# eniac/flamingo

Hardware: AMD Instinct MI355X
Metric: device-resident aggregate+unmask GB/s, N clients × L int32 per round (higher is better)
Workload: dtype u32

## Files before the change

flamingo_amd/csrc/flm_internal.h:

```cpp
#pragma once
#include <stdint.h>
#include <stddef.h>
#include <hip/hip_runtime.h>

#include "flm_host_layout.h"
#include "flm_items.h"

namespace flm {

constexpr uint32_t kAbcd = 0x64636261u;
constexpr uint32_t kSigma0 = 0x61707865u, kSigma1 = 0x3320646eu, kSigma2 = 0x79622d32u,
                   kSigma3 = 0x6b206574u;

hipError_t launch_seed_schedule(const uint8_t *d_seeds, const int8_t *d_signs, int K, SeedRec *d_recs,
                                uint32_t *d_meta, hipStream_t stream, uint32_t *d_zero = nullptr,
                                uint64_t zero_n = 0);
int seed_schedule_groups(int K, uint64_t zero_n);
hipError_t launch_items(int subtiles, int variant, const Item *d_items, int n_items, const uint32_t *d_rows,
                        uint64_t row_pitch, const SeedRec *d_recs, const uint32_t *d_meta,
                        uint32_t *d_out, hipStream_t stream);
int small_round_slots(int B);
hipError_t launch_small_round(int B, const uint32_t *d_rows, uint64_t pitch, int N, const uint8_t *d_seeds,
                              const int8_t *d_signs, int K, uint64_t L, uint64_t mask_lo, uint64_t mask_hi,
                              uint32_t ctr0, uint32_t *d_out, uint32_t *d_meta, hipStream_t stream);
hipError_t launch_small_client_mask(const uint32_t *d_x, uint64_t pitch, int N, const int64_t *d_seg,
                                   const uint8_t *d_seeds, const int8_t *d_signs, uint64_t L, uint32_t bias,
                                   uint32_t *d_out, hipStream_t stream);
uint32_t pair_units_count(int K, uint64_t L, uint32_t *n_tiles);
hipError_t launch_pair_units(bool side, const SeedRec *d_recs, int K, uint32_t *d_dst, uint64_t L, uint32_t *d_ws,
                             int groups, hipStream_t stream);
hipError_t launch_flag_set(uint32_t *d_ws, hipStream_t stream);
hipError_t launch_prg_expand(const SeedRec *d_recs, int K, uint64_t L, uint64_t pitch, uint32_t ctr0,
                             uint32_t *d_out, int groups, hipStream_t stream);
hipError_t launch_add2(const uint32_t *d_a, const uint32_t *d_b, uint32_t *d_dst, uint64_t n, hipStream_t stream);
constexpr int kMaxParts = 16;
struct PartPtrs {
    const uint32_t *p[kMaxParts];
};
hipError_t launch_shard_sum(const uint32_t *const *d_parts, int G, uint64_t lo, uint64_t n, uint32_t *d_dst,
                            hipStream_t stream);
hipError_t launch_chacha20_xor(const uint32_t key[8], const uint32_t nonce[2], uint64_t counter,
                               const uint8_t *d_in, uint8_t *d_out, size_t n, hipStream_t stream);

// ... 70 lines not shown
```

flamingo_amd/csrc/flm_kernels.hip:

```cpp
#include "flm_internal.h"

namespace flm {

#define FLM_ROTL(v, c) __builtin_rotateleft32((v), (c))
#define FLM_QR(a, b, c, d)                       \
    a += b; d ^= a; d = FLM_ROTL(d, 16);          \
    c += d; b ^= c; b = FLM_ROTL(b, 12);          \
    a += b; d ^= a; d = FLM_ROTL(d, 8);           \
    c += d; b ^= c; b = FLM_ROTL(b, 7);

#define FLM_GAP_A1 ""
#define FLM_GAP_AX ""
#define FLM_GAP_X1 ""
#define FLM_GAP_XR ""
#define FLM_GAP_R0 "s_nop 1\n\t"
#define FLM_GAP_R1 "s_nop 1\n\t"
#define FLM_GAP_R2 "s_nop 1\n\t"
#define FLM_GAP_RA "s_nop 2\n\t"
#define FLM_S_A(a, b) "v_add_u32 %[" #a "], %[" #b "], %[" #a "]\n\t"
#define FLM_S_X(a, b) "v_xor_b32 %[" #a "], %[" #b "], %[" #a "]\n\t"
#define FLM_S_R(a, s) "v_alignbit_b32 %[" #a "], %[" #a "], %[" #a "], " #s "\n\t"
#define FLM_S_STEP(a, b, c, d, s)                                                                       \
    FLM_S_A(a##0, b##0) FLM_S_A(a##1, b##1) FLM_GAP_A1 FLM_S_A(a##2, b##2) FLM_S_A(a##3, b##3) FLM_GAP_AX \
    FLM_S_X(d##0, a##0) FLM_S_X(d##1, a##1) FLM_GAP_X1 FLM_S_X(d##2, a##2) FLM_S_X(d##3, a##3) FLM_GAP_XR \
// ... 54 lines not shown
#pragma unroll
        for (int i = 0; i < 10; ++i) r.pad[i] = 0;
        recs[k] = r;
    }
    __shared__ uint32_t s_cnt[2][4];
    const unsigned long long bn = __ballot(neg != 0), bb = __ballot(bad != 0);
    const int w = threadIdx.x >> 6;
    if ((threadIdx.x & 63) == 0) { s_cnt[0][w] = __popcll(bn); s_cnt[1][w] = __popcll(bb); }
    __syncthreads();
    if (threadIdx.x == 0) {
        meta[2 + 2 * blockIdx.x] = s_cnt[0][0] + s_cnt[0][1] + s_cnt[0][2] + s_cnt[0][3];
        meta[3 + 2 * blockIdx.x] = s_cnt[1][0] + s_cnt[1][1] + s_cnt[1][2] + s_cnt[1][3];
        if (blockIdx.x == 0) meta[0] = gridDim.x;
    }
}

__device__ __forceinline__ uint32_t meta_nneg(const uint32_t *__restrict__ meta) {
    const uint32_t parts = meta[0];
    uint32_t n = 0;
    for (uint32_t p = 0; p < parts; ++p) n += meta[2 + 2 * p];
    return n;
}

__device__ __forceinline__ void chacha_mask_add(const SeedRec *__restrict__ rec, uint32_t ctr,
                                                uint32_t (&m)[16]) {
    const uint32_t k0 = rec->k[0], k1 = rec->k[1], k2 = rec->k[2], k3 = rec->k[3];
    const uint32_t k4 = rec->k[4], k5 = rec->k[5], k6 = rec->k[6], k7 = rec->k[7];
    const uint32_t xc = rec->xorc;
    uint32_t x0, x1, x2, x3, x4, x5, x6, x7, x8, x9, x10, x11, x12, x13, x14, x15;
    x0 = rec->a0;
    x12 = FLM_ROTL(ctr ^ x0, 16);
    x8 = k4 + x12;
    x4 = FLM_ROTL(k0 ^ x8, 12);
    x0 += x4;
    x12 = FLM_ROTL(x12 ^ x0, 8);
    x8 += x12;
    x4 = FLM_ROTL(x4 ^ x8, 7);
    x1 = rec->col1[0]; x5 = rec->col1[1]; x9 = rec->col1[2]; x13 = rec->col1[3];
    x2 = rec->col2[0]; x6 = rec->col2[1]; x10 = rec->col2[2]; x14 = rec->col2[3];
    x3 = rec->col3[0]; x7 = rec->col3[1]; x11 = rec->col3[2]; x15 = rec->col3[3];
    FLM_QR4(x0, x5, x10, x15, x1, x6, x11, x12, x2, x7, x8, x13, x3, x4, x9, x14);
#pragma unroll
    for (int r = 0; r < 9; ++r) {
        FLM_QR4(x0, x4, x8, x12, x1, x5, x9, x13, x2, x6, x10, x14, x3, x7, x11, x15);
        FLM_QR4(x0, x5, x10, x15, x1, x6, x11, x12, x2, x7, x8, x13, x3, x4, x9, x14);
    }
    m[0] += (x0 + kSigma0) ^ xc;
    m[1] += (x1 + kSigma1) ^ xc;
    m[2] += (x2 + kSigma2) ^ xc;
    m[3] += (x3 + kSigma3) ^ xc;
    m[4] += (x4 + k0) ^ xc;
    m[5] += (x5 + k1) ^ xc;
    m[6] += (x6 + k2) ^ xc;
    m[7] += (x7 + k3) ^ xc;
    m[8] += (x8 + k4) ^ xc;
    m[9] += (x9 + k5) ^ xc;
    m[10] += (x10 + k6) ^ xc;
    m[11] += (x11 + k7) ^ xc;
    m[12] += (x12 + ctr) ^ xc;
    m[13] += x13 ^ xc;
    m[14] += x14 ^ xc;
    m[15] += x15 ^ xc;
}

typedef uint32_t u32x4 __attribute__((ext_vector_type(4)));

template <bool BL, int AUX = 0>
__device__ __forceinline__ void load_row(const uint32_t *base, uint32_t bytes, int lane, u32x4 (&v)[4]) {
    const __amdgpu_buffer_rsrc_t rs = __builtin_amdgcn_make_buffer_rsrc(const_cast<uint32_t *>(base), 0,
                                                                        (int)bytes, 0x00020000);
#pragma unroll
    for (int j = 0; j < 4; ++j)
        v[j] = __builtin_bit_cast(
            u32x4, __builtin_amdgcn_raw_buffer_load_b128(rs, BL ? 64 * lane + 16 * j : 16 * lane + 1024 * j, 0, AUX));
}

template <int S>
__device__ __forceinline__ void reduce_out(const u32x4 *__restrict__ lds, uint32_t *__restrict__ out,
                                           uint64_t base, int valid, uint32_t bias, bool atomic) {
    constexpr int Cw = kWavesPerGroup / S;
    if (!atomic) {
        for (int q = threadIdx.x; q < S * 256; q += kThreads) {
            const int s = q >> 8, p = q & 255;
            u32x4 acc = u32x4(bias);
#pragma unroll
            for (int c = 0; c < Cw; ++c) acc = acc + lds[(s + S * c) * 256 + p];
            const int slot = s * kWaveSlots + 4 * p;
            uint32_t *dst = out + base + slot;
            if (slot + 3 < valid) {
                *reinterpret_cast<u32x4 *>(dst) = acc;
            } else {
                if (slot + 0 < valid) dst[0] = acc.x;
                if (slot + 1 < valid) dst[1] = acc.y;
                if (slot + 2 < valid) dst[2] = acc.z;
            }
        }
    } else {
        const uint32_t *l32 = reinterpret_cast<const uint32_t *>(lds);
        for (int d = threadIdx.x; d < S * kWaveSlots; d += kThreads) {
            const int s = d >> 10, o = d & 1023;
            uint32_t acc = bias;
#pragma unroll
            for (int c = 0; c < Cw; ++c) acc += l32[(s + S * c) * 1024 + o];
            const int slot = s * kWaveSlots + o;
            if (slot < valid) atomicAdd(out + base + slot, acc);
        }
    }
}

template <int S, bool BL, bool MERGED, int WPE, int RUM = 2, int AUX = 0, bool SPREAD = false>
__global__ __launch_bounds__(kThreads, WPE) void items_kernel(const Item *__restrict__ items,
                                                              const uint32_t *__restrict__ rows,
                                                              uint64_t row_pitch,
                                                              const SeedRec *__restrict__ recs,
                                                              const uint32_t *__restrict__ meta,
                                                              uint32_t *__restrict__ out) {
    static_assert(!MERGED || BL, "merged accumulation needs block-layout rows");
    constexpr int Cw = kWavesPerGroup / S;
    constexpr int RU = MERGED ? RUM : 4;
    __shared__ u32x4 lds[kWavesPerGroup * 256];
    __shared__ uint32_t claim[S];

    const Item it = items[blockIdx.x];
    const int lane = threadIdx.x & 63;
    const int w = __builtin_amdgcn_readfirstlane(threadIdx.x >> 6);
    const int s = w % S, c = w / S;
    if constexpr (!SPREAD && Cw > 1) {
        if (threadIdx.x < S) claim[threadIdx.x] = 0u;
        __syncthreads();
    }
    const uint32_t flags = it.flags;
    const bool has_rows = flags & kHasRows, has_mask = flags & kHasMask;

    u32x4 racc[4] = {u32x4(0u), u32x4(0u), u32x4(0u), u32x4(0u)};
    uint32_t m[16];
#pragma unroll
    for (int i = 0; i < 16; ++i) m[i] = 0;

    uint32_t nr = 0, ns = 0, r0 = 0, q0 = 0;
    if (has_rows) {
        r0 = (uint32_t)(((uint64_t)it.nrows * c) / Cw);
        nr = (uint32_t)(((uint64_t)it.nrows * (c + 1)) / Cw) - r0;
    }
    if (has_mask) {
        q0 = it.k0 + (uint32_t)(((uint64_t)it.nseeds * c) / Cw);
        ns = it.k0 + (uint32_t)(((uint64_t)it.nseeds * (c + 1)) / Cw) - q0;
    }
    const int sub_slot = s * kWaveSlots;
    const int row_valid = (int)it.row_valid - sub_slot;
    const uint32_t row_bytes =
        row_valid >= kWaveSlots ? 4u * kWaveSlots : (row_valid > 0 ? 16u * (uint32_t)((row_valid + 3) / 4) : 0u);
    const uint32_t *rp = rows + it.row_in + (uint64_t)r0 * row_pitch + sub_slot;
    const uint32_t ctr = (uint32_t)(it.mask_ctr + (uint64_t)(sub_slot / 16) + (uint64_t)lane);
    const SeedRec *rec = recs + q0;
    if (row_valid <= 0) nr = 0;

    auto add_row = [&](const u32x4 (&v)[4]) {
        if constexpr (MERGED) {
#pragma unroll
            for (int j = 0; j < 4; ++j) {
                m[4 * j + 0] += v[j].x; m[4 * j + 1] += v[j].y; m[4 * j + 2] += v[j].z; m[4 * j + 3] += v[j].w;
            }
        } else {
#pragma unroll
            for (int j = 0; j < 4; ++j) racc[j] = racc[j] + v[j];
        }
    };

    if constexpr (SPREAD) {
        uint32_t q = 0;
        for (uint32_t r = 0; r < nr; ++r) {
            u32x4 v[4];
            load_row<BL, AUX>(rp, row_bytes, lane, v);
            if (q < ns && (uint64_t)q * nr <= (uint64_t)r * ns) {
                chacha_mask_add(rec, ctr, m);
                ++rec;
                ++q;
            }
            add_row(v);
            rp += row_pitch;
        }
        for (; q < ns; ++q) {
            chacha_mask_add(rec, ctr, m);
            ++rec;
        }
    } else if constexpr (Cw > 1) {
        const uint32_t NR = (has_rows && row_valid > 0) ? it.nrows : 0u;
        const uint32_t NS = has_mask ? it.nseeds : 0u;
        const uint32_t *rb = rows + it.row_in + sub_slot;
        const uint32_t caddr = (uint32_t)(uintptr_t)(__attribute__((address_space(3))) uint32_t *)&claim[s];
        auto next = [&]() -> uint32_t {
            uint32_t v = 0;
            if (lane == 0)
                asm volatile("ds_add_rtn_u32 %0, %1, %2\n\ts_waitcnt lgkmcnt(0)" : "=v"(v) : "v"(caddr), "v"(1u) : "memory");
            return __builtin_amdgcn_readlane(v, 0);
        };
        const uint32_t NP = NR < NS ? NR : NS;
        uint32_t i = next();
        for (; i < NP; i = next()) {
            u32x4 v4[4];
            load_row<BL, AUX>(rb + (uint64_t)i * row_pitch, row_bytes, lane, v4);
            chacha_mask_add(recs + it.k0 + i, ctr, m);
            add_row(v4);
        }
        for (; i < NS; i = next()) chacha_mask_add(recs + it.k0 + i, ctr, m);
        if (NR > NS) {
            const uint32_t a = NS + (uint32_t)(((uint64_t)(NR - NS) * c) / Cw);
            const uint32_t b = NS + (uint32_t)(((uint64_t)(NR - NS) * (c + 1)) / Cw);
            const uint32_t *rq = rb + (uint64_t)a * row_pitch;
            uint32_t rr = b - a;
            for (; rr >= RU; rr -= RU) {
                u32x4 v4[RU][4];
#pragma unroll
                for (int u = 0; u < RU; ++u) load_row<BL, AUX>(rq + u * row_pitch, row_bytes, lane, v4[u]);
#pragma unroll
                for (int u = 0; u < RU; ++u) add_row(v4[u]);
                rq += RU * row_pitch;
            }
            for (; rr > 0; --rr) {
                u32x4 v4[4];
                load_row<BL, AUX>(rq, row_bytes, lane, v4);
                add_row(v4);
                rq += row_pitch;
            }
        }
    } else {
        const uint32_t np = nr < ns ? nr : ns;
        for (uint32_t q = 0; q < np; ++q) {
            u32x4 v[4];
            load_row<BL, AUX>(rp, row_bytes, lane, v);
            chacha_mask_add(rec, ctr, m);
            add_row(v);
            rp += row_pitch;
            ++rec;
        }
        uint32_t rr = nr - np;
        for (; rr >= RU; rr -= RU) {
            u32x4 v[RU][4];
#pragma unroll
            for (int u = 0; u < RU; ++u) load_row<BL, AUX>(rp + u * row_pitch, row_bytes, lane, v[u]);
#pragma unroll
            for (int u = 0; u < RU; ++u) add_row(v[u]);
            rp += RU * row_pitch;
        }
        for (; rr > 0; --rr) {
            u32x4 v[4];
            load_row<BL, AUX>(rp, row_bytes, lane, v);
            add_row(v);
            rp += row_pitch;
        }
        for (uint32_t q = np; q < ns; ++q) {
            chacha_mask_add(rec, ctr, m);
            ++rec;
        }
    }

    u32x4 *R = lds + w * 256;
    const uint32_t mbias = it.mask_bias + ((flags & kMaskBiasNneg) ? meta_nneg(meta) : 0u);
    if constexpr (MERGED) {
        R[4 * lane + 0] = u32x4{m[0], m[1], m[2], m[3]};
        R[4 * lane + 1] = u32x4{m[4], m[5], m[6], m[7]};
        R[4 * lane + 2] = u32x4{m[8], m[9], m[10], m[11]};
        R[4 * lane + 3] = u32x4{m[12], m[13], m[14], m[15]};
        __syncthreads();
        const uint64_t base = has_mask ? it.mask_out : it.row_out;
        const int valid = has_mask ? (int)it.mask_valid : (int)it.row_valid;
        const uint32_t bias = (has_rows ? it.row_bias : 0u) + (has_mask ? mbias : 0u);
        reduce_out<S>(lds, out, base, valid, bias, (flags & (kRowAtomic | kMaskAtomic)) != 0);
    } else {
        const bool same = flags & kSameTile;
        u32x4 mq[4];
        if (has_mask) {
            if (BL) {
                mq[0] = u32x4{m[0], m[1], m[2], m[3]};
                mq[1] = u32x4{m[4], m[5], m[6], m[7]};
                mq[2] = u32x4{m[8], m[9], m[10], m[11]};
                mq[3] = u32x4{m[12], m[13], m[14], m[15]};
            } else {
                R[4 * lane + 0] = u32x4{m[0], m[1], m[2], m[3]};
                R[4 * lane + 1] = u32x4{m[4], m[5], m[6], m[7]};
                R[4 * lane + 2] = u32x4{m[8], m[9], m[10], m[11]};
// ... 345 lines not shown
}

#undef FLM_QR
#undef FLM_ROTL

int seed_schedule_groups(int K, uint64_t zero_n) {
    const uint64_t g = (uint64_t)((K + 255) / 256 > 0 ? (K + 255) / 256 : 1);
    const uint64_t z = std::min<uint64_t>(1024, (zero_n + 4095) / 4096);
    return (int)std::max(g, z);
}

hipError_t launch_seed_schedule(const uint8_t *d_seeds, const int8_t *d_signs, int K, SeedRec *d_recs,
                                uint32_t *d_meta, hipStream_t stream, uint32_t *d_zero, uint64_t zero_n) {
    const unsigned grid = (unsigned)seed_schedule_groups(K, d_zero ? zero_n : 0);
    hipLaunchKernelGGL(seed_schedule_kernel, dim3(grid), dim3(256), 0, stream, d_seeds, d_signs, K, d_recs, d_meta,
                       d_zero, d_zero ? zero_n : 0);
    return hipGetLastError();
}

template <int S, bool BL, bool MERGED, int WPE, int RUM = 2, int AUX = 0, bool SPREAD = false>
static void launch_items_t(const Item *d_items, int n_items, const uint32_t *d_rows, uint64_t row_pitch,
                           const SeedRec *d_recs, const uint32_t *d_meta, uint32_t *d_out, hipStream_t stream) {
    hipLaunchKernelGGL((items_kernel<S, BL, MERGED, WPE, RUM, AUX, SPREAD>), dim3(n_items), dim3(kThreads), 0, stream, d_items, d_rows,
                       row_pitch, d_recs, d_meta, d_out);
}

hipError_t launch_items(int subtiles, int variant, const Item *d_items, int n_items, const uint32_t *d_rows,
                        uint64_t row_pitch, const SeedRec *d_recs, const uint32_t *d_meta, uint32_t *d_out,
                        hipStream_t stream) {
    if (n_items <= 0) return hipSuccess;
#define FLM_L(S, BL, MG, W, ...) \
    launch_items_t<S, BL, MG, W, ##__VA_ARGS__>(d_items, n_items, d_rows, row_pitch, d_recs, d_meta, d_out, stream)
#define FLM_V(S)                                                     \
    switch (variant) {                                               \
        case kVarCoalesced: FLM_L(S, false, false, 4); break;        \
        case kVarBlock: FLM_L(S, true, false, 4); break;             \
        case kVarMerged: FLM_L(S, true, true, 4, 2, 0); break;           \
        case kVarMergedW8: FLM_L(S, true, true, 8); break;           \
        case kVarMergedRU4: FLM_L(S, true, true, 4, 4, 0); break;    \
        case kVarMergedNT: FLM_L(S, true, true, 4, 2, 2); break;     \
        case kVarMergedRU4NT: FLM_L(S, true, true, 4, 4, 2); break;  \
        case kVarMergedSpread: FLM_L(S, true, true, 4, 2, 0, true); break; \
        case kVarBlockSpread: FLM_L(S, true, false, 4, 2, 0, true); break; \
        default: return hipErrorInvalidValue;                        \
    }
    switch (subtiles) {
        case 1: FLM_V(1) break;
// ... 106 lines not shown
```

flamingo_amd/csrc/flm_runtime.hip:

```cpp
#include <hip/hip_runtime.h>
#include <hip/hip_ext.h>

#include <algorithm>
#include <cassert>
#include <cstdarg>
#include <cstdio>
#include <cstdlib>
#include <cstring>
#include <map>
#include <string>
#include <tuple>
#include <vector>

#include "../../include/flamingo_hip.h"
#include "flm_copy_pool.h"
#include "flm_deal_args.h"
#include "flm_ecdsa_args.h"
#include "flm_feldman_args.h"
#include "flm_internal.h"
#include "flm_planner.h"

using flm::Item;
using flm::SeedRec;
using flm::plan::PlanShape;
// ... 120 lines not shown
    DevBuf recs, meta;
    hipEvent_t written = nullptr;
    bool written_valid = false;
    hipStream_t w_stream = nullptr;
    StreamMarks readers;
    uint64_t last_use = 0;
};

}

constexpr int kSmallRoundVariant = 100;
constexpr int kExpandVariant = 101;

struct flm_ctx {
    int device = 0;
    hipStream_t stream = nullptr;
    std::string err;
    DevBuf rows, out, seeds, signs, bytes_in, bytes_out;
    std::vector<SeedTable *> tables;
    SeedTable *cur_table = nullptr;
    SeedTable *pub_table = nullptr;
    DevBuf small_meta;
    bool last_small = false;
    uint64_t table_clock = 0;
    std::vector<StageSlot *> slots;
    uint64_t slot_clock = 0;
    DevBuf ec_in, ec_base, ec_scal, ec_jac, ec_out, ec_dig, ec_flags;
    void *stage[2] = {nullptr, nullptr};
    size_t stage_cap = 0;
    hipEvent_t stage_done[2] = {nullptr, nullptr};
    hipStream_t copy[4] = {nullptr, nullptr, nullptr, nullptr};
    hipEvent_t copy_done[4] = {nullptr, nullptr, nullptr, nullptr};
    hipEvent_t copy_start = nullptr;
    std::map<PlanKey, Plan *> plans;
    uint64_t plan_clock = 0;
    int last_items = 0, last_tile = 0, last_atomics = 0, last_variant = 0;
    int table_k = -1;
    int tune_variant = -1;
    int tune_subtiles = 0;
    int tune_min_items = flm::plan::kDefaultMinItems;
    int tune_ec_threads = 64;
    int tune_ec_waves = 1;
    int tune_ec_spread = 0;
    int tune_ec_terms = 1;
    int tune_ec_coop = -1;
    int tune_small = 1;
    int tune_pairing = 1;
    int tune_expand_waves = 128;
    int n_cus = 0;
    void *bounce = nullptr;
    void *bounce_dev = nullptr;
    size_t bounce_cap = 0;
    CopyPool copies;
    void *comm = nullptr;
};

namespace {

int fail(flm_ctx *ctx, int code, const char *fmt, ...) {
    char buf[512];
    va_list ap;
    va_start(ap, fmt);
    vsnprintf(buf, sizeof buf, fmt, ap);
    va_end(ap);
    if (ctx) ctx->err = buf;
    g_last_error = buf;
    return code;
}

#define FLM_ON_DEVICE(ctx)                 \
    flm::rt::DeviceScope dev_scope_;       \
    FLM_HIP((ctx), dev_scope_.set((ctx)->device))

#define FLM_HIP(ctx, expr)                                                                            \
    do {                                                                                              \
        hipError_t e_ = (expr);                                                                       \
        if (e_ != hipSuccess)                                                                         \
            return fail((ctx), FLM_EHIP, "%s failed: %s (%s:%d)", #expr, hipGetErrorString(e_), __FILE__, \
                        __LINE__);                                                                    \
    } while (0)

inline uint64_t round_up(uint64_t v, uint64_t m) { return (v + m - 1) / m * m; }

struct TuneKey {
    const char *name;
    int flm_ctx::*member;
    bool (*accepts)(int);
    const char *refusal;
};
template <int Lo, int Hi> bool within(int v) { return v >= Lo && v <= Hi; }
template <int... V> bool one_of(int v) { return ((v == V) || ...); }
const TuneKey kTuneKeys[] = {
    {"variant", &flm_ctx::tune_variant, within<-1, flm::kVarCount - 1>, "variant %d out of range"},
    {"pairing", &flm_ctx::tune_pairing, within<0, 2>, "pairing must be 0, 1 or 2"},
    {"subtiles", &flm_ctx::tune_subtiles, one_of<0, 1, 4, 16>, "subtiles must be 0 (auto), 1, 4 or 16"},
    {"ec_waves", &flm_ctx::tune_ec_waves, one_of<1, 4, 8>, "ec_waves must be 1, 4 or 8"},
    {"small", &flm_ctx::tune_small, within<0, 2>, "small must be 0 (never), 1 (auto) or 2 (when legal)"},
    {"min_items", &flm_ctx::tune_min_items, within<64, 1 << 20>, "min_items must be in [64, 2^20]"},
    {"ec_spread", &flm_ctx::tune_ec_spread, within<0, 64>, "ec_spread must be in [0, 64] KiB"},
    {"ec_terms", &flm_ctx::tune_ec_terms, one_of<1, 2, 4>, "ec_terms must be 1, 2 or 4"},
    {"ec_coop", &flm_ctx::tune_ec_coop, within<-1, 2>, "ec_coop must be -1, 0, 1 or 2"},
    {"expand_waves", &flm_ctx::tune_expand_waves, within<1, 256>, "expand_waves must be in [1, 256]"},
    {"ec_threads", &flm_ctx::tune_ec_threads, one_of<64, 128, 256>, "ec_threads must be 64, 128 or 256"},
};
const TuneKey *tune_key(const char *key) {
    for (const TuneKey &t : kTuneKeys)
        if (!std::strcmp(key, t.name)) return &t;
    return nullptr;
}

void set_last_plan(flm_ctx *ctx, int items, int tile_slots, int atomics, int variant) {
    ctx->last_items = items, ctx->last_tile = tile_slots, ctx->last_atomics = atomics, ctx->last_variant = variant;
}

StageSlot *stage_acquire(flm_ctx *ctx, size_t bytes, int *rc) {
    StageSlot *best = nullptr, *free_small = nullptr, *oldest = nullptr;
    for (StageSlot *s : ctx->slots) {
        if (s->busy && event_done(s->done)) s->busy = false;
        if (s->busy) {
            if (!oldest || s->last < oldest->last) oldest = s;
// ... 101 lines not shown
Plan *aggregate_plan(flm_ctx *ctx, uint64_t pitch, int N, int K, uint64_t L, uint64_t mask_lo, uint64_t mask_hi,
                     uint64_t prg_slot0, hipStream_t s, int *rc) {
    PlanKey key{ctx->tune_subtiles + 100 * ctx->tune_pairing + 1000 * ctx->tune_min_items, pitch, (uint64_t)N,
                (uint64_t)K, L, mask_lo, mask_hi, prg_slot0};
    auto f = ctx->plans.find(key);
    if (f != ctx->plans.end()) {
        f->second->last_use = ++ctx->plan_clock;
        *rc = 0;
        return f->second;
    }
    Plan *plan = nullptr;
    if (ctx->plans.size() >= kPlanCache) {
        auto lru = ctx->plans.begin();
        for (auto it = ctx->plans.begin(); it != ctx->plans.end(); ++it)
            if (it->second->last_use < lru->second->last_use) lru = it;
        Plan *old = lru->second;
        hipError_t e = old->done.sync_all();
        if (e == hipSuccess && old->ready) e = hipEventSynchronize(old->ready);
        if (e != hipSuccess) {
            *rc = fail(ctx, FLM_EHIP, "plan cache: waiting for a recycled plan failed: %s", hipGetErrorString(e));
            return nullptr;
        }
        ctx->plans.erase(lru);
        plan = new Plan();
        plan->items = old->items;
        plan->ready = old->ready;
        plan->done.swap(old->done);
        delete old;
    } else {
        plan = new Plan();
    }
    std::vector<Item> items;
    plan->shape = flm::plan::build_aggregate_items(ctx->tune_subtiles, ctx->tune_pairing, pitch, N, K, L, mask_lo, mask_hi,
                                                   prg_slot0, items, ctx->tune_min_items);
    *rc = upload_plan(ctx, *plan, items, s);
    if (*rc) { plan_free(plan); return nullptr; }
    plan->last_use = ++ctx->plan_clock;
    ctx->plans[key] = plan;
    return plan;
}

bool signs_ok(const int8_t *signs, int K, int *nneg) {
    int n = 0;
    for (int k = 0; k < K; ++k) {
        if (signs[k] == -1) ++n;
        else if (signs[k] != 1) return false;
// ... 39 lines not shown
            return nullptr;
        }
    }
    hipError_t e = t->recs.reserve(std::max<size_t>(1, (size_t)K) * sizeof(SeedRec));
    if (e == hipSuccess) e = t->meta.reserve(sizeof(uint32_t) * std::max<size_t>(4, meta_words));
    if (e != hipSuccess) {
        *rc = fail(ctx, FLM_ENOMEM, "seed table of %d seeds: %s", K, hipGetErrorString(e));
        return nullptr;
    }
    t->last_use = ++ctx->table_clock;
    if (ctx->pub_table == t) {
        ctx->pub_table = nullptr;
        ctx->table_k = -1;
    }
    *rc = 0;
    return t;
}

hipError_t table_written(flm_ctx *ctx, SeedTable *t, hipStream_t s, bool record) {
    t->w_stream = s;
    t->written_valid = record;
    ctx->cur_table = t;
    ctx->last_small = false;
    return record ? hipEventRecord(t->written, s) : hipSuccess;
}

void table_cover(SeedTable *t, hipStream_t s) {
    if (t && !t->written_valid && hipEventRecord(t->written, s) == hipSuccess) t->written_valid = true;
    (void)hipGetLastError();
}

hipError_t table_before_read(SeedTable *t, hipStream_t s) {
    if (t->w_stream == s) return hipSuccess;
    if (t->written_valid) return event_done(t->written) ? hipSuccess : hipStreamWaitEvent(s, t->written, 0);
    const hipEvent_t read = t->readers.event_of(t->w_stream);
    return read ? hipStreamWaitEvent(s, read, 0) : hipSuccess;
}

hipError_t table_read(SeedTable *t, hipStream_t s) { return t->readers.record(s); }

void table_free(SeedTable *t) {
    if (t->written && t->written_valid) (void)hipEventSynchronize(t->written);
    (void)t->readers.sync_all();
    t->recs.release();
    t->meta.release();
    if (t->written) (void)hipEventDestroy(t->written);
    delete t;
}

int run_small_round(flm_ctx *ctx, int B, const uint32_t *d_rows, uint64_t pitch, int N, const uint8_t *d_seeds,
                    const int8_t *d_signs, int K, uint64_t L, uint64_t mask_lo, uint64_t mask_hi, uint64_t prg_slot0,
                    uint32_t *d_out, hipStream_t s) {
    FLM_HIP(ctx, ctx->small_meta.reserve(4 * sizeof(uint32_t)));
    FLM_HIP(ctx, flm::launch_small_round(B, d_rows, pitch, N, d_seeds, d_signs, K, L, mask_lo, mask_hi,
                                         (uint32_t)(prg_slot0 / 16), d_out, ctx->small_meta.as<uint32_t>(), s));
    ctx->last_small = true;
    ctx->pub_table = nullptr;
    ctx->table_k = -1;
    return 0;
}

int run_seed_schedule(flm_ctx *ctx, const uint8_t *d_seeds, const int8_t *d_signs, int K, hipStream_t s,
                      SeedTable **out, uint32_t *zero_out = nullptr, uint64_t zero_n = 0, bool publish = false) {
    const int groups = flm::seed_schedule_groups(K, zero_out ? zero_n : 0);
    int rc = 0;
    SeedTable *t = table_acquire(ctx, K, 2 + 2 * (size_t)groups, s, &rc);
    if (!t) return rc;
    const hipError_t e = flm::launch_seed_schedule(d_seeds, d_signs, K, t->recs.as<SeedRec>(), t->meta.as<uint32_t>(),
                                                   s, zero_out, zero_n);
    if (e != hipSuccess) {
        table_cover(t, s);
        return fail(ctx, FLM_EHIP, "seed schedule launch: %s", hipGetErrorString(e));
    }
    FLM_HIP(ctx, table_written(ctx, t, s, publish));
    ctx->pub_table = publish ? t : nullptr;
    ctx->table_k = publish ? K : -1;
    *out = t;
    return 0;
}

int run_plan(flm_ctx *ctx, Plan &plan, SeedTable *table, const uint32_t *d_rows, uint64_t pitch, uint32_t *d_out,
             size_t out_elems, hipStream_t s, bool zeroed = false) {
    if (!plan.ready_known) {
        if (event_done(plan.ready)) plan.ready_known = true;
        else if (s != plan.up_stream) FLM_HIP(ctx, hipStreamWaitEvent(s, plan.ready, 0));
    }
    if (plan.shape.needs_zero && !zeroed) FLM_HIP(ctx, hipMemsetAsync(d_out, 0, out_elems * sizeof(uint32_t), s));
    const int variant_id = flm::plan::pick_variant(ctx->tune_variant, plan.shape);
    FLM_HIP(ctx, table_before_read(table, s));
    FLM_HIP(ctx, flm::launch_items(plan.shape.subtiles, variant_id, plan.items.as<Item>(), plan.n_items, d_rows, pitch,
                                   table->recs.as<SeedRec>(), table->meta.as<uint32_t>(), d_out, s));
    FLM_HIP(ctx, table_read(table, s));
    FLM_HIP(ctx, plan.done.record(s));
    set_last_plan(ctx, plan.n_items, flm::kWaveSlots * plan.shape.subtiles, plan.shape.atomics, variant_id);
    return 0;
}

bool host_pinned(const void *p) {
    hipPointerAttribute_t a;
    const hipError_t e = hipPointerGetAttributes(&a, p);
    if (e != hipSuccess) {
        (void)hipGetLastError();
        return false;
    }
    return a.type == hipMemoryTypeHost;
}

using flm::rt::kStageBytes;
using flm::rt::Piece;
using flm::rt::pieces;

int ensure_stage(flm_ctx *ctx) {
    if (ctx->stage_cap >= kStageBytes) return 0;
    for (int b = 0; b < 2; ++b) {
        if (ctx->stage[b]) (void)hipHostFree(ctx->stage[b]);
        ctx->stage[b] = nullptr;
// ... 319 lines not shown
    e = hipStreamCreateWithFlags(&ctx->stream, hipStreamNonBlocking);
    if (e != hipSuccess) {
        delete ctx;
        return fail(nullptr, FLM_EHIP, "hipStreamCreate: %s", hipGetErrorString(e));
    }
    if (hipDeviceGetAttribute(&ctx->n_cus, hipDeviceAttributeMultiprocessorCount, device) != hipSuccess) {
        (void)hipGetLastError();
        ctx->n_cus = 256;
    }
    stage_prealloc(ctx);
    *out = ctx;
    return 0;
}

void flm_free(flm_ctx *ctx) {
    if (!ctx) return;
    flm::rt::DeviceScope dev_scope_(ctx->device);
    if (ctx->stream) (void)hipStreamSynchronize(ctx->stream);
    if (ctx->comm) (void)hipDeviceSynchronize();
    flm::comm_release(ctx);
    for (StageSlot *s : ctx->slots) (void)hipEventSynchronize(s->done);
    for (auto &kv : ctx->plans) plan_free(kv.second);
    for (SeedTable *t : ctx->tables) table_free(t);
    if (ctx->small_meta.p) (void)hipDeviceSynchronize();
    ctx->small_meta.release();
    for (DevBuf *b : {&ctx->rows, &ctx->out, &ctx->seeds, &ctx->signs, &ctx->bytes_in, &ctx->bytes_out, &ctx->ec_in,
                      &ctx->ec_base, &ctx->ec_scal, &ctx->ec_jac, &ctx->ec_out, &ctx->ec_dig, &ctx->ec_flags})
        b->release();
    for (StageSlot *s : ctx->slots) {
        if (s->host) (void)hipHostFree(s->host);
        s->dev.release();
        (void)hipEventDestroy(s->done);
        delete s;
    }
    if (ctx->bounce) (void)hipHostFree(ctx->bounce);
    for (int i = 0; i < 2; ++i) {
        if (ctx->stage[i]) (void)hipHostFree(ctx->stage[i]);
        if (ctx->stage_done[i]) (void)hipEventDestroy(ctx->stage_done[i]);
    }
    for (int c = 0; c < 4; ++c) {
        if (ctx->copy[c]) (void)hipStreamSynchronize(ctx->copy[c]);
        if (ctx->copy[c]) (void)hipStreamDestroy(ctx->copy[c]);
        if (ctx->copy_done[c]) (void)hipEventDestroy(ctx->copy_done[c]);
    }
    if (ctx->copy_start) (void)hipEventDestroy(ctx->copy_start);
    if (ctx->stream) (void)hipStreamDestroy(ctx->stream);
    delete ctx;
}
// ... 68 lines not shown
    return run_plan(ctx, *plan, ctx->pub_table, d_rows, row_pitch, d_out, L, s);
}

int flm_aggregate_unmask_dev(flm_ctx *ctx, const uint32_t *d_rows, size_t row_pitch, int N, const uint8_t *d_seeds,
                             const int8_t *d_signs, int K, size_t L, size_t mask_lo, size_t mask_hi,
                             uint64_t prg_slot0, uint32_t *d_out, void *stream) {
    if (!ctx) return fail(nullptr, FLM_EINVAL, "ctx is NULL");
    if (L == 0) return 0;
    if (int rc = check_aggregate_args(ctx, d_rows, row_pitch, N, K, L, mask_lo, mask_hi, prg_slot0, d_out)) return rc;
    if (K > 0 && (!d_seeds || !d_signs)) return fail(ctx, FLM_EINVAL, "seeds/signs NULL");
    hipStream_t s = static_cast<hipStream_t>(stream);
    FLM_ON_DEVICE(ctx);
    int rc = 0;
    if (const int B = flm::plan::small_round_width(ctx->tune_small, N, K, L, mask_lo, mask_hi)) {
        if ((rc = run_small_round(ctx, B, d_rows, row_pitch, N, d_seeds, d_signs, K, L, mask_lo, mask_hi, prg_slot0,
                                  d_out, s)))
            return rc;
        const int slots = flm::small_round_slots(B);
        set_last_plan(ctx, (int)((L + slots - 1) / slots), slots, 0, kSmallRoundVariant);
        return 0;
    }
    Plan *plan = aggregate_plan(ctx, row_pitch, N, K, L, mask_lo, mask_hi, prg_slot0, s, &rc);
    if (!plan) return rc;
    SeedTable *table = nullptr;
    if ((rc = run_seed_schedule(ctx, d_seeds, d_signs, K, s, &table, plan->shape.needs_zero ? d_out : nullptr, L))) return rc;
    if ((rc = run_plan(ctx, *plan, table, d_rows, row_pitch, d_out, L, s, plan->shape.needs_zero))) table_cover(table, s);
    return rc;
}

int flm_client_mask(flm_ctx *ctx, const uint32_t *x, int N, const int64_t *seg, const uint8_t *seeds,
                    const int8_t *signs, size_t L, uint32_t *out) {
    if (!ctx) return fail(nullptr, FLM_EINVAL, "ctx is NULL");
    if (N < 0) return fail(ctx, FLM_EINVAL, "negative N");
    if (N == 0 || L == 0) return 0;
    if (!seg || !out) return fail(ctx, FLM_EINVAL, "NULL argument");
    if (seg[0] != 0) return fail(ctx, FLM_EINVAL, "seg[0] must be 0");
    for (int i = 0; i < N; ++i)
        if (seg[i + 1] < seg[i]) return fail(ctx, FLM_EINVAL, "seg must be non-decreasing");
    const int64_t K = seg[N];
    if (K > 0 && (!seeds || !signs)) return fail(ctx, FLM_EINVAL, "NULL seeds/signs");
    if (K > 0x7fffffff) return fail(ctx, FLM_EINVAL, "too many seeds");
    if (!signs_ok(signs, (int)K, nullptr)) return fail(ctx, FLM_EINVAL, "signs must be +1 or -1");
    if (int rc = check_range(ctx, 0, L)) return rc;
    FLM_ON_DEVICE(ctx);
    const uint64_t pitch = round_up(L, 64);
    HostCopies hc(ctx, ctx->stream);
// ... 169 lines not shown
}

int flm_set_tuning(flm_ctx *ctx, const char *key, int value) {
    if (!ctx || !key) return fail(ctx, FLM_EINVAL, "NULL argument");
    const TuneKey *t = tune_key(key);
    if (!t) return fail(ctx, FLM_EINVAL, "unknown tuning key '%s'", key);
    if (!t->accepts(value)) return fail(ctx, FLM_EINVAL, t->refusal, value);
    ctx->*t->member = value;
    return 0;
}

int flm_get_tuning(const flm_ctx *ctx, const char *key, int *value) {
    flm_ctx *c = const_cast<flm_ctx *>(ctx);
    if (!ctx || !key || !value) return fail(c, FLM_EINVAL, "NULL argument");
    const TuneKey *t = tune_key(key);
    if (!t) return fail(c, FLM_EINVAL, "unknown tuning key '%s'", key);
    *value = ctx->*t->member;
    return 0;
}

int flm_check_signs(flm_ctx *ctx, int *bad_count) {
    if (!ctx || !bad_count) return fail(ctx, FLM_EINVAL, "NULL argument");
    *bad_count = 0;
    const SeedTable *t = ctx->last_small ? nullptr : ctx->cur_table;
    const DevBuf *meta = ctx->last_small ? &ctx->small_meta : (t ? &t->meta : nullptr);
    if (!meta || !meta->p) return 0;
    FLM_ON_DEVICE(ctx);
    if (t && t->written_valid) FLM_HIP(ctx, hipEventSynchronize(t->written));
    if (const hipEvent_t read = t ? t->readers.event_of(t->w_stream) : nullptr) FLM_HIP(ctx, hipEventSynchronize(read));
    uint32_t parts = 0;
    FLM_HIP(ctx, hipMemcpy(&parts, meta->p, sizeof parts, hipMemcpyDeviceToHost));
    if (2 + 2 * (size_t)parts > meta->cap / sizeof(uint32_t))
        return fail(ctx, FLM_EHIP, "seed table sign counts: %u parts overrun the table", parts);
    std::vector<uint32_t> m(2 + 2 * (size_t)parts);
    FLM_HIP(ctx, hipMemcpy(m.data(), meta->p, m.size() * sizeof(uint32_t), hipMemcpyDeviceToHost));
    for (uint32_t p = 0; p < parts; ++p) *bad_count += (int)m[3 + 2 * p];
    return 0;
}

int flm_last_plan(const flm_ctx *ctx, int *items, int *tile_slots, int *atomics, int *variant) {
    if (!ctx) return FLM_EINVAL;
    if (items) *items = ctx->last_items;
    if (tile_slots) *tile_slots = ctx->last_tile;
    if (atomics) *atomics = ctx->last_atomics;
    if (variant) *variant = ctx->last_variant;
    return 0;
// ... 514 lines not shown
```

flamingo_amd/distributed.py:

```python
from __future__ import annotations

import torch
import torch.distributed as dist

SHARD_ALIGN = 1024


def padded_length(L: int, world: int) -> int:
    q = SHARD_ALIGN * world
    return (L + q - 1) // q * q


def shard_bounds(L: int, world: int, rank: int):
    S = padded_length(L, world) // world
    lo = min(rank * S, L)
    hi = min((rank + 1) * S, L)
    return lo, hi


def client_bounds(N: int, world: int, rank: int):
    return N * rank // world, N * (rank + 1) // world


def init_rccl(engine, group=None):
# ... 69 lines not shown
        if self.force_collective and not dist.is_initialized():
            raise RuntimeError("force_collective needs an initialised torch.distributed group")
        self._solo = self.world == 1 and not self.force_collective
        self.L = L
        self.Lp = padded_length(L, self.world)
        self.S = self.Lp // self.world
        self.lo, self.hi = shard_bounds(L, self.world, self.rank)
        dev = device if device is not None else torch.device("cuda", torch.cuda.current_device())
        if buffers not in (1, 2):
            raise ValueError("buffers must be 1 or 2")
        if comm is None:
            comm = "rccl" if (engine is not None and not self._solo and engine.has_comm()
                              and engine.comm_size() == (self.world, self.rank)) else "torch"
        if comm not in ("rccl", "torch"):
            raise ValueError("comm must be 'rccl' or 'torch'")
        if comm == "rccl" and (not engine.has_comm() or engine.comm_size() != (self.world, self.rank)):
            raise RuntimeError("comm='rccl' needs init_rccl(engine, group) first")
        self.comm = comm
        self._partials = [torch.zeros(self.Lp, dtype=torch.int32, device=dev) for _ in range(buffers)]
        self._outs = [torch.empty(self.S, dtype=torch.int32, device=dev) for _ in range(buffers)]
        self._pending = [None] * buffers
        self._comm_stream = torch.cuda.Stream(device=dev) if (comm == "rccl" and buffers == 2) else None
        self._k = 0
        self.partial, self.out = self._partials[0], self._outs[0]

    def prepare_seeds(self, d_seeds, d_signs, stream=None):
        self.K = d_seeds.shape[0]
        self.engine.seed_table_dev(d_seeds, d_signs, stream=stream)

    def compute(self, d_rows, stream=None):
        self.engine.aggregate_dev(d_rows, self.K, self.partial, L=self.L, mask_lo=self.lo, mask_hi=self.hi,
                                  stream=stream)

    def _torch_exchange(self, async_op: bool = False):
        if self.partial.is_cuda and dist.get_backend(self.group) == "gloo":
            cpu_out = torch.empty(self.out.shape, dtype=self.out.dtype)
            dist.reduce_scatter_tensor(cpu_out, self.partial.cpu(), op=dist.ReduceOp.SUM, group=self.group)
            self.out.copy_(cpu_out)
            return None
        return dist.reduce_scatter_tensor(self.out, self.partial, op=dist.ReduceOp.SUM, group=self.group,
                                          async_op=async_op)

    def exchange(self, stream=None):
        if self._solo:
            return self.partial[: self.L]
        if self.comm == "rccl":
            self.engine.reduce_scatter_dev(self.partial, self.out, self.S, stream=stream)
        else:
            st = _torch_stream(stream)
            if st is not None and self.partial.is_cuda:
                with torch.cuda.stream(st):
                    self._torch_exchange()
            else:
                self._torch_exchange()
        return self.out[: self.hi - self.lo]

    def step(self, d_rows, d_seeds, d_signs, stream=None):
        self.prepare_seeds(d_seeds, d_signs, stream)
        self.compute(d_rows, stream)
        return self.exchange(stream)

    def _async_ok(self):
        if self._solo:
            return False
        if self.comm == "rccl":
            return self._comm_stream is not None
        return not (self.partial.is_cuda and dist.get_backend(self.group) == "gloo")

    def launch(self, d_rows, d_seeds, d_signs, stream=None) -> int:
        b = self._k % len(self._partials)
        st = _torch_stream(stream)
        if self._pending[b] is not None:
            if self.comm == "rccl":
                (st or torch.cuda.current_stream()).wait_event(self._pending[b])
            elif st is not None and self.partial.is_cuda:
                with torch.cuda.stream(st):
                    self._pending[b].wait()
            else:
                self._pending[b].wait()
            self._pending[b] = None
        self.partial, self.out = self._partials[b], self._outs[b]
        self.prepare_seeds(d_seeds, d_signs, stream)
        self.compute(d_rows, stream)
        if not self._async_ok():
            self.exchange(stream)
        elif self.comm == "rccl":
            ready = torch.cuda.Event()
            ready.record(st or torch.cuda.current_stream())
            self._comm_stream.wait_event(ready)
            self.engine.reduce_scatter_dev(self.partial, self.out, self.S, stream=self._comm_stream)
            done = torch.cuda.Event()
            done.record(self._comm_stream)
            self._pending[b] = done
        elif st is not None and self.partial.is_cuda:
            with torch.cuda.stream(st):
                self._pending[b] = self._torch_exchange(async_op=True)
        else:
            self._pending[b] = self._torch_exchange(async_op=True)
        self._k += 1
        return b

    def result(self, b: int | None = None):
        b = (self._k - 1) % len(self._partials) if b is None else b
        if self._pending[b] is not None:
            if self.comm == "rccl":
                torch.cuda.current_stream().wait_event(self._pending[b])
# ... 7 lines not shown
```

Baseline: 3202.

## Derive seed records inside the items kernel instead of a separate schedule pass

Adds a RAW variant of the items kernel that reads raw seeds and signs directly. Each wave computes the key-dependent ChaCha first-column quarter-rounds and the sign-dependent constants itself, and counts negative and invalid signs in-kernel. This removes the separate seed-schedule launch and the SeedRec table round trip from each aggregate round, and the Python wrapper routes through a combined aggregate_unmask path. The cost is redundant per-wave precomputation of the seed record, extra kernel arguments, and a diagnostic atomic plus ring buffer for sign checks.

```diff
diff --git a/flamingo_amd/csrc/flm_internal.h b/flamingo_amd/csrc/flm_internal.h
--- a/flamingo_amd/csrc/flm_internal.h
+++ b/flamingo_amd/csrc/flm_internal.h
@@ -19,6 +19,15 @@
 hipError_t launch_items(int subtiles, int variant, const Item *d_items, int n_items, const uint32_t *d_rows,
                         uint64_t row_pitch, const SeedRec *d_recs, const uint32_t *d_meta,
                         uint32_t *d_out, hipStream_t stream);
+struct RawSeeds {
+    const uint8_t *seeds;
+    const int8_t *signs;
+    uint64_t first_ctr;
+    uint32_t *diag;
+};
+bool items_raw_built(int subtiles, int variant, const uint8_t *d_seeds);
+hipError_t launch_items_raw(int subtiles, int variant, const Item *d_items, int n_items, const uint32_t *d_rows,
+                            uint64_t row_pitch, const RawSeeds &raw, uint32_t *d_out, hipStream_t stream);
 int small_round_slots(int B);
 hipError_t launch_small_round(int B, const uint32_t *d_rows, uint64_t pitch, int N, const uint8_t *d_seeds,
                               const int8_t *d_signs, int K, uint64_t L, uint64_t mask_lo, uint64_t mask_hi,
diff --git a/flamingo_amd/csrc/flm_kernels.hip b/flamingo_amd/csrc/flm_kernels.hip
--- a/flamingo_amd/csrc/flm_kernels.hip
+++ b/flamingo_amd/csrc/flm_kernels.hip
@@ -100,7 +100,8 @@
     return n;
 }
 
-__device__ __forceinline__ void chacha_mask_add(const SeedRec *__restrict__ rec, uint32_t ctr,
+template <class Rec>
+__device__ __forceinline__ void chacha_mask_add(const Rec *__restrict__ rec, uint32_t ctr,
                                                 uint32_t (&m)[16]) {
     const uint32_t k0 = rec->k[0], k1 = rec->k[1], k2 = rec->k[2], k3 = rec->k[3];
     const uint32_t k4 = rec->k[4], k5 = rec->k[5], k6 = rec->k[6], k7 = rec->k[7];
@@ -141,6 +142,47 @@
     m[15] += x15 ^ xc;
 }
 
+struct RawRec {
+    uint32_t k[8], xorc, a0, col1[4], col2[4], col3[4];
+};
+
+#define FLM_SROTL(v, c) ((uint32_t)(((((uint64_t)(v)) << 32) | (uint64_t)(v)) >> (32 - (c))))
+#define FLM_SQR(a, b, c, d)                        \
+    a += b; d ^= a; d = FLM_SROTL(d, 16);          \
+    c += d; b ^= c; b = FLM_SROTL(b, 12);          \
+    a += b; d ^= a; d = FLM_SROTL(d, 8);           \
+    c += d; b ^= c; b = FLM_SROTL(b, 7);
+
+__device__ __forceinline__ void raw_rec(const uint32_t *__restrict__ seeds, const uint32_t *__restrict__ signs,
+                                        uint32_t sign_off, uint32_t q, RawRec &r, uint32_t &neg, uint32_t &bad) {
+    const uint32_t *p = seeds + 8 * (uint64_t)q;
+#pragma unroll
+    for (int i = 0; i < 8; ++i) r.k[i] = p[i];
+    const uint32_t e = sign_off + q;
+    const int sg = (int)(int8_t)(signs[e >> 2] >> (8 * (e & 3)));
+    neg = sg < 0 ? 1u : 0u;
+    bad = (sg != 1 && sg != -1) ? 1u : 0u;
+    r.xorc = sg < 0 ? ~kAbcd : kAbcd;
+    r.a0 = kSigma0 + r.k[0];
+    uint32_t x1 = kSigma1, x5 = r.k[1], x9 = r.k[5], x13 = 0u;
+    uint32_t x2 = kSigma2, x6 = r.k[2], x10 = r.k[6], x14 = 0u;
+    uint32_t x3 = kSigma3, x7 = r.k[3], x11 = r.k[7], x15 = 0u;
+    FLM_SQR(x1, x5, x9, x13);
+    FLM_SQR(x2, x6, x10, x14);
+    FLM_SQR(x3, x7, x11, x15);
+#define FLM_SPIN(v) asm("" : "+s"(v))
+    FLM_SPIN(x1); FLM_SPIN(x5); FLM_SPIN(x9); FLM_SPIN(x13);
+    FLM_SPIN(x2); FLM_SPIN(x6); FLM_SPIN(x10); FLM_SPIN(x14);
+    FLM_SPIN(x3); FLM_SPIN(x7); FLM_SPIN(x11); FLM_SPIN(x15);
+    FLM_SPIN(r.a0);
+#undef FLM_SPIN
+    r.col1[0] = x1; r.col1[1] = x5; r.col1[2] = x9; r.col1[3] = x13;
+    r.col2[0] = x2; r.col2[1] = x6; r.col2[2] = x10; r.col2[3] = x14;
+    r.col3[0] = x3; r.col3[1] = x7; r.col3[2] = x11; r.col3[3] = x15;
+}
+#undef FLM_SQR
+#undef FLM_SROTL
+
 typedef uint32_t u32x4 __attribute__((ext_vector_type(4)));
 
 template <bool BL, int AUX = 0>
@@ -186,13 +228,17 @@
     }
 }
 
-template <int S, bool BL, bool MERGED, int WPE, int RUM = 2, int AUX = 0, bool SPREAD = false>
+template <int S, bool BL, bool MERGED, int WPE, int RUM = 2, int AUX = 0, bool SPREAD = false, bool RAW = false>
 __global__ __launch_bounds__(kThreads, WPE) void items_kernel(const Item *__restrict__ items,
                                                               const uint32_t *__restrict__ rows,
                                                               uint64_t row_pitch,
                                                               const SeedRec *__restrict__ recs,
                                                               const uint32_t *__restrict__ meta,
-                                                              uint32_t *__restrict__ out) {
+                                                              uint32_t *__restrict__ out,
+                                                              const uint32_t *__restrict__ raw_seeds,
+                                                              const uint32_t *__restrict__ raw_signs,
+                                                              uint32_t sign_off, uint64_t first_ctr,
+                                                              uint32_t *__restrict__ diag) {
     static_assert(!MERGED || BL, "merged accumulation needs block-layout rows");
     constexpr int Cw = kWavesPerGroup / S;
     constexpr int RU = MERGED ? RUM : 4;
@@ -233,6 +279,20 @@
     const SeedRec *rec = recs + q0;
     if (row_valid <= 0) nr = 0;
 
+    uint32_t nneg = 0, nbad = 0;
+    auto mask_add = [&](const SeedRec *r, uint32_t q) {
+        if constexpr (RAW) {
+            RawRec rr;
+            uint32_t neg, bad;
+            raw_rec(raw_seeds, raw_signs, sign_off, q, rr, neg, bad);
+            nneg += neg;
+            nbad += bad;
+            chacha_mask_add(&rr, ctr, m);
+        } else {
+            chacha_mask_add(r, ctr, m);
+        }
+    };
+
     auto add_row = [&](const u32x4 (&v)[4]) {
         if constexpr (MERGED) {
 #pragma unroll
@@ -251,7 +311,7 @@
             u32x4 v[4];
             load_row<BL, AUX>(rp, row_bytes, lane, v);
             if (q < ns && (uint64_t)q * nr <= (uint64_t)r * ns) {
-                chacha_mask_add(rec, ctr, m);
+                mask_add(rec, q0 + q);
                 ++rec;
                 ++q;
             }
@@ -259,7 +319,7 @@
             rp += row_pitch;
         }
         for (; q < ns; ++q) {
-            chacha_mask_add(rec, ctr, m);
+            mask_add(rec, q0 + q);
             ++rec;
         }
     } else if constexpr (Cw > 1) {
@@ -278,10 +338,10 @@
         for (; i < NP; i = next()) {
             u32x4 v4[4];
             load_row<BL, AUX>(rb + (uint64_t)i * row_pitch, row_bytes, lane, v4);
-            chacha_mask_add(recs + it.k0 + i, ctr, m);
+            mask_add(recs + it.k0 + i, it.k0 + i);
             add_row(v4);
         }
-        for (; i < NS; i = next()) chacha_mask_add(recs + it.k0 + i, ctr, m);
+        for (; i < NS; i = next()) mask_add(recs + it.k0 + i, it.k0 + i);
         if (NR > NS) {
             const uint32_t a = NS + (uint32_t)(((uint64_t)(NR - NS) * c) / Cw);
             const uint32_t b = NS + (uint32_t)(((uint64_t)(NR - NS) * (c + 1)) / Cw);
@@ -307,7 +367,7 @@
         for (uint32_t q = 0; q < np; ++q) {
             u32x4 v[4];
             load_row<BL, AUX>(rp, row_bytes, lane, v);
-            chacha_mask_add(rec, ctr, m);
+            mask_add(rec, q0 + q);
             add_row(v);
             rp += row_pitch;
             ++rec;
@@ -328,13 +388,20 @@
             rp += row_pitch;
         }
         for (uint32_t q = np; q < ns; ++q) {
-            chacha_mask_add(rec, ctr, m);
+            mask_add(rec, q0 + q);
             ++rec;
         }
     }
 
     u32x4 *R = lds + w * 256;
-    const uint32_t mbias = it.mask_bias + ((flags & kMaskBiasNneg) ? meta_nneg(meta) : 0u);
+    uint32_t mbias = it.mask_bias;
+    if constexpr (RAW) {
+#pragma unroll
+        for (int i = 0; i < 16; ++i) m[i] += nneg;
+        if (s == 0 && has_mask && it.mask_ctr == first_ctr && nbad != 0u && lane == 0) atomicAdd(diag, nbad);
+    } else {
+        mbias += (flags & kMaskBiasNneg) ? meta_nneg(meta) : 0u;
+    }
     if constexpr (MERGED) {
         R[4 * lane + 0] = u32x4{m[0], m[1], m[2], m[3]};
         R[4 * lane + 1] = u32x4{m[4], m[5], m[6], m[7]};
@@ -726,7 +793,41 @@
 static void launch_items_t(const Item *d_items, int n_items, const uint32_t *d_rows, uint64_t row_pitch,
                            const SeedRec *d_recs, const uint32_t *d_meta, uint32_t *d_out, hipStream_t stream) {
     hipLaunchKernelGGL((items_kernel<S, BL, MERGED, WPE, RUM, AUX, SPREAD>), dim3(n_items), dim3(kThreads), 0, stream, d_items, d_rows,
-                       row_pitch, d_recs, d_meta, d_out);
+                       row_pitch, d_recs, d_meta, d_out, (const uint32_t *)nullptr, (const uint32_t *)nullptr, 0u,
+                       (uint64_t)0, (uint32_t *)nullptr);
+}
+
+template <int S, bool MERGED, bool SPREAD>
+static void launch_items_raw_t(const Item *d_items, int n_items, const uint32_t *d_rows, uint64_t row_pitch,
+                               const RawSeeds &raw, uint32_t *d_out, hipStream_t stream) {
+    const uintptr_t sa = (uintptr_t)raw.signs;
+    hipLaunchKernelGGL((items_kernel<S, true, MERGED, 4, 2, 0, SPREAD, true>), dim3(n_items), dim3(kThreads), 0, stream,
+                       d_items, d_rows, row_pitch, (const SeedRec *)nullptr, (const uint32_t *)nullptr, d_out,
+                       reinterpret_cast<const uint32_t *>(raw.seeds), reinterpret_cast<const uint32_t *>(sa & ~(uintptr_t)3),
+                       (uint32_t)(sa & 3), raw.first_ctr, raw.diag);
+}
+
+bool items_raw_built(int subtiles, int variant, const uint8_t *d_seeds) {
+    if (((uintptr_t)d_seeds & 3) != 0 || (subtiles != 1 && subtiles != 4)) return false;
+    return variant == kVarMerged || variant == kVarMergedSpread || variant == kVarBlock || variant == kVarBlockSpread;
+}
+
+hipError_t launch_items_raw(int subtiles, int variant, const Item *d_items, int n_items, const uint32_t *d_rows,
+                            uint64_t row_pitch, const RawSeeds &raw, uint32_t *d_out, hipStream_t stream) {
+    if (!items_raw_built(subtiles, variant, raw.seeds)) return hipErrorInvalidValue;
+    if (n_items <= 0) return hipSuccess;
+#define FLM_R(S, MG, SP) launch_items_raw_t<S, MG, SP>(d_items, n_items, d_rows, row_pitch, raw, d_out, stream)
+#define FLM_RV(S)                                            \
+    switch (variant) {                                       \
+        case kVarBlock: FLM_R(S, false, false); break;       \
+        case kVarMerged: FLM_R(S, true, false); break;       \
+        case kVarMergedSpread: FLM_R(S, true, true); break;  \
+        default: FLM_R(S, false, true); break;               \
+    }
+    if (subtiles == 1) { FLM_RV(1) } else { FLM_RV(4) }
+#undef FLM_RV
+#undef FLM_R
+    return hipGetLastError();
 }
 
 hipError_t launch_items(int subtiles, int variant, const Item *d_items, int n_items, const uint32_t *d_rows,
diff --git a/flamingo_amd/csrc/flm_runtime.hip b/flamingo_amd/csrc/flm_runtime.hip
--- a/flamingo_amd/csrc/flm_runtime.hip
+++ b/flamingo_amd/csrc/flm_runtime.hip
@@ -166,6 +166,12 @@
     SeedTable *pub_table = nullptr;
     DevBuf small_meta;
     bool last_small = false;
+    DevBuf raw_diag;
+    uint64_t raw_seq = 0;
+    int last_raw = 0;
+    int raw_word = 0;
+    Plan *raw_plan = nullptr;
+    hipStream_t raw_stream = nullptr;
     uint64_t table_clock = 0;
     std::vector<StageSlot *> slots;
     uint64_t slot_clock = 0;
@@ -189,6 +195,7 @@
     int tune_ec_terms = 1;
     int tune_ec_coop = -1;
     int tune_small = 1;
+    int tune_raw = 1;
     int tune_pairing = 1;
     int tune_expand_waves = 128;
     int n_cus = 0;
@@ -234,12 +241,15 @@
 };
 template <int Lo, int Hi> bool within(int v) { return v >= Lo && v <= Hi; }
 template <int... V> bool one_of(int v) { return ((v == V) || ...); }
+bool read_only(int) { return false; }
 const TuneKey kTuneKeys[] = {
     {"variant", &flm_ctx::tune_variant, within<-1, flm::kVarCount - 1>, "variant %d out of range"},
     {"pairing", &flm_ctx::tune_pairing, within<0, 2>, "pairing must be 0, 1 or 2"},
     {"subtiles", &flm_ctx::tune_subtiles, one_of<0, 1, 4, 16>, "subtiles must be 0 (auto), 1, 4 or 16"},
     {"ec_waves", &flm_ctx::tune_ec_waves, one_of<1, 4, 8>, "ec_waves must be 1, 4 or 8"},
     {"small", &flm_ctx::tune_small, within<0, 2>, "small must be 0 (never), 1 (auto) or 2 (when legal)"},
+    {"raw", &flm_ctx::tune_raw, within<0, 1>, "raw must be 0 (seed table) or 1 (in-kernel seed records)"},
+    {"last_raw", &flm_ctx::last_raw, read_only, "last_raw is read-only"},
     {"min_items", &flm_ctx::tune_min_items, within<64, 1 << 20>, "min_items must be in [64, 2^20]"},
     {"ec_spread", &flm_ctx::tune_ec_spread, within<0, 64>, "ec_spread must be in [0, 64] KiB"},
     {"ec_terms", &flm_ctx::tune_ec_terms, one_of<1, 2, 4>, "ec_terms must be 1, 2 or 4"},
@@ -387,6 +397,7 @@
             return nullptr;
         }
         ctx->plans.erase(lru);
+        if (ctx->raw_plan == old) ctx->raw_plan = nullptr;
         plan = new Plan();
         plan->items = old->items;
         plan->ready = old->ready;
@@ -472,6 +483,7 @@
     t->written_valid = record;
     ctx->cur_table = t;
     ctx->last_small = false;
+    ctx->last_raw = 0;
     return record ? hipEventRecord(t->written, s) : hipSuccess;
 }
 
@@ -505,6 +517,7 @@
     FLM_HIP(ctx, flm::launch_small_round(B, d_rows, pitch, N, d_seeds, d_signs, K, L, mask_lo, mask_hi,
                                          (uint32_t)(prg_slot0 / 16), d_out, ctx->small_meta.as<uint32_t>(), s));
     ctx->last_small = true;
+    ctx->last_raw = 0;
     ctx->pub_table = nullptr;
     ctx->table_k = -1;
     return 0;
@@ -542,6 +555,34 @@
                                    table->recs.as<SeedRec>(), table->meta.as<uint32_t>(), d_out, s));
     FLM_HIP(ctx, table_read(table, s));
     FLM_HIP(ctx, plan.done.record(s));
+    set_last_plan(ctx, plan.n_items, flm::kWaveSlots * plan.shape.subtiles, plan.shape.atomics, variant_id);
+    return 0;
+}
+
+constexpr size_t kRawDiagWords = 1024;
+int run_plan_raw(flm_ctx *ctx, Plan &plan, int variant_id, const uint32_t *d_rows, uint64_t pitch, const uint8_t *d_seeds,
+                 const int8_t *d_signs, uint64_t first_slot, uint32_t *d_out, size_t out_elems, hipStream_t s) {
+    FLM_HIP(ctx, ctx->raw_diag.reserve(kRawDiagWords * sizeof(uint32_t)));
+    const size_t word = (size_t)(ctx->raw_seq % kRawDiagWords);
+    if (word % (kRawDiagWords / 2) == 0)
+        FLM_HIP(ctx, hipMemsetAsync(ctx->raw_diag.as<uint32_t>() + word, 0, kRawDiagWords / 2 * sizeof(uint32_t), s));
+    ++ctx->raw_seq;
+    if (!plan.ready_known) {
+        if (event_done(plan.ready)) plan.ready_known = true;
+        else if (s != plan.up_stream) FLM_HIP(ctx, hipStreamWaitEvent(s, plan.ready, 0));
+    }
+    if (plan.shape.needs_zero) FLM_HIP(ctx, hipMemsetAsync(d_out, 0, out_elems * sizeof(uint32_t), s));
+    const flm::RawSeeds raw{d_seeds, d_signs, first_slot / 16, ctx->raw_diag.as<uint32_t>() + word};
+    FLM_HIP(ctx, flm::launch_items_raw(plan.shape.subtiles, variant_id, plan.items.as<Item>(), plan.n_items, d_rows, pitch,
+                                       raw, d_out, s));
+    FLM_HIP(ctx, plan.done.record(s));
+    ctx->raw_word = (int)word;
+    ctx->raw_plan = &plan;
+    ctx->raw_stream = s;
+    ctx->last_raw = 1;
+    ctx->last_small = false;
+    ctx->pub_table = nullptr;
+    ctx->table_k = -1;
     set_last_plan(ctx, plan.n_items, flm::kWaveSlots * plan.shape.subtiles, plan.shape.atomics, variant_id);
     return 0;
 }
@@ -907,8 +948,10 @@
     for (StageSlot *s : ctx->slots) (void)hipEventSynchronize(s->done);
     for (auto &kv : ctx->plans) plan_free(kv.second);
     for (SeedTable *t : ctx->tables) table_free(t);
-    if (ctx->small_meta.p) (void)hipDeviceSynchronize();
+    if (ctx->small_meta.p || ctx->raw_diag.p) (void)hipDeviceSynchronize();
     ctx->small_meta.release();
+    ctx->raw_diag.release();
+    ctx->raw_plan = nullptr;
     for (DevBuf *b : {&ctx->rows, &ctx->out, &ctx->seeds, &ctx->signs, &ctx->bytes_in, &ctx->bytes_out, &ctx->ec_in,
                       &ctx->ec_base, &ctx->ec_scal, &ctx->ec_jac, &ctx->ec_out, &ctx->ec_dig, &ctx->ec_flags})
         b->release();
@@ -1023,6 +1066,9 @@
     }
     Plan *plan = aggregate_plan(ctx, row_pitch, N, K, L, mask_lo, mask_hi, prg_slot0, s, &rc);
     if (!plan) return rc;
+    const int variant_id = flm::plan::pick_variant(ctx->tune_variant, plan->shape);
+    if (ctx->tune_raw && (K == 0 || mask_hi > mask_lo) && flm::items_raw_built(plan->shape.subtiles, variant_id, d_seeds))
+        return run_plan_raw(ctx, *plan, variant_id, d_rows, row_pitch, d_seeds, d_signs, prg_slot0 + mask_lo, d_out, L, s);
     SeedTable *table = nullptr;
     if ((rc = run_seed_schedule(ctx, d_seeds, d_signs, K, s, &table, plan->shape.needs_zero ? d_out : nullptr, L))) return rc;
     if ((rc = run_plan(ctx, *plan, table, d_rows, row_pitch, d_out, L, s, plan->shape.needs_zero))) table_cover(table, s);
@@ -1238,6 +1284,16 @@
 int flm_check_signs(flm_ctx *ctx, int *bad_count) {
     if (!ctx || !bad_count) return fail(ctx, FLM_EINVAL, "NULL argument");
     *bad_count = 0;
+    if (ctx->last_raw) {
+        if (!ctx->raw_diag.p) return 0;
+        FLM_ON_DEVICE(ctx);
+        if (const hipEvent_t done = ctx->raw_plan ? ctx->raw_plan->done.event_of(ctx->raw_stream) : nullptr)
+            FLM_HIP(ctx, hipEventSynchronize(done));
+        uint32_t bad = 0;
+        FLM_HIP(ctx, hipMemcpy(&bad, ctx->raw_diag.as<uint32_t>() + ctx->raw_word, sizeof bad, hipMemcpyDeviceToHost));
+        *bad_count = (int)bad;
+        return 0;
+    }
     const SeedTable *t = ctx->last_small ? nullptr : ctx->cur_table;
     const DevBuf *meta = ctx->last_small ? &ctx->small_meta : (t ? &t->meta : nullptr);
     if (!meta || !meta->p) return 0;
diff --git a/flamingo_amd/distributed.py b/flamingo_amd/distributed.py
--- a/flamingo_amd/distributed.py
+++ b/flamingo_amd/distributed.py
@@ -115,13 +115,32 @@
         self._pending = [None] * buffers
         self._comm_stream = torch.cuda.Stream(device=dev) if (comm == "rccl" and buffers == 2) else None
         self._k = 0
+        self._seeds = None
+        self._handing = False
         self.partial, self.out = self._partials[0], self._outs[0]
 
     def prepare_seeds(self, d_seeds, d_signs, stream=None):
         self.K = d_seeds.shape[0]
+        if self._handing:
+            self._seeds = (d_seeds, d_signs)
+            return
+        self._seeds = None
         self.engine.seed_table_dev(d_seeds, d_signs, stream=stream)
 
+    def _round(self, d_rows, d_seeds, d_signs, stream):
+        self._handing = True
+        try:
+            self.prepare_seeds(d_seeds, d_signs, stream)
+        finally:
+            self._handing = False
+        self.compute(d_rows, stream)
+
     def compute(self, d_rows, stream=None):
+        seeds, self._seeds = self._seeds, None
+        if seeds is not None:
+            self.engine.aggregate_unmask_dev(d_rows, seeds[0], seeds[1], self.partial, L=self.L, mask_lo=self.lo,
+                                             mask_hi=self.hi, stream=stream)
+            return
         self.engine.aggregate_dev(d_rows, self.K, self.partial, L=self.L, mask_lo=self.lo, mask_hi=self.hi,
                                   stream=stream)
 
@@ -149,8 +168,7 @@
         return self.out[: self.hi - self.lo]
 
     def step(self, d_rows, d_seeds, d_signs, stream=None):
-        self.prepare_seeds(d_seeds, d_signs, stream)
-        self.compute(d_rows, stream)
+        self._round(d_rows, d_seeds, d_signs, stream)
         return self.exchange(stream)
 
     def _async_ok(self):
@@ -173,8 +191,7 @@
                 self._pending[b].wait()
             self._pending[b] = None
         self.partial, self.out = self._partials[b], self._outs[b]
-        self.prepare_seeds(d_seeds, d_signs, stream)
-        self.compute(d_rows, stream)
+        self._round(d_rows, d_seeds, d_signs, stream)
         if not self._async_ok():
             self.exchange(stream)
         elif self.comm == "rccl":
```

New measurement: 3219, median of 6. No clear change (+0.5%).
